# baudm/parseq

Hardware: AMD Instinct MI355X
Metric: images/sec (32x128 crops) PARSeq-S AR+refine (higher is better)
Workload: dtype bf16x3

## Files before the change

parseq_amd/csrc/decoder_attn.h:

```cpp
#pragma once
#include "common.h"

namespace pq {

constexpr int DEC_MAXL = 32;
constexpr int DEC_HD = 32;

template <typename T>
__global__ __launch_bounds__(256)
void score_table_kernel(const float* __restrict__ qself, const T* __restrict__ kvtab, float* __restrict__ stab,
                        int npos, int ntok, int E) {
    const int H = E / DEC_HD;
    const size_t total = (size_t)npos * npos * ntok * H;
    const size_t idx = (size_t)blockIdx.x * blockDim.x + threadIdx.x;
    if (idx >= total) return;
    const int h = (int)(idx % H);
    size_t r = idx / H;
    const int tok = (int)(r % ntok); r /= ntok;
    const int j = (int)(r % npos);
    const int i = (int)(r / npos);
    const float* q = qself + (size_t)i * E + h * DEC_HD;
    const T* k = kvtab + ((size_t)j * ntok + tok) * (2 * E) + h * DEC_HD;
    float s = 0.f;
#pragma unroll
// ... 246 lines not shown
__device__ __forceinline__ float f24_even(unsigned hw, unsigned lw, int i) {
    return __uint_as_float(__builtin_amdgcn_perm(hw, lw, 0x0504000cu | ((unsigned)(i & 3) << 8)));
}
__device__ __forceinline__ float f24_odd(unsigned hw, unsigned lw, int i) {
    return __uint_as_float(__builtin_amdgcn_perm(hw, lw, 0x0706000cu | ((unsigned)(i & 3) << 8)));
}
__device__ __forceinline__ void f24_unpack8(const u32x4& hi, const uint2& lo, float (&v)[8]) {
#pragma unroll
    for (int i = 0; i < 8; i += 2) {
        const unsigned lw = i < 4 ? lo.x : lo.y;
        v[i] = f24_even(hi[i >> 1], lw, i);
        v[i + 1] = f24_odd(hi[i >> 1], lw, i + 1);
    }
}

template <int E, bool QSPLIT = false>
__global__ __launch_bounds__(E)
void dec_cross_attn_ar24_kernel(const float* __restrict__ qc, const QAsm qa, const unsigned char* __restrict__ kmem, const unsigned char* __restrict__ vmem,
                                size_t plane_elems, float scale, float* __restrict__ out) {
    constexpr int H = E / DEC_HD, NK = 128, LPR = 4, KPL = 16, NL = 8;
    const int lane = threadIdx.x & 63, wid = threadIdx.x >> 6, nw = E / 64, b = blockIdx.x;
    const int kl = lane / LPR, dl = lane % LPR;
    auto over_keys_sum = [](float v) {
        v = dpp_add<0x124>(v);
        v = dpp_add<0x128>(v);
        v += __shfl_xor(v, 16, 64);
        v += __shfl_xor(v, 32, 64);
        return v;
    };
    auto over_keys_max = [](float v) {
        v = dpp_max<0x124>(v);
        v = dpp_max<0x128>(v);
        v = fmaxf(v, __shfl_xor(v, 16, 64));
        v = fmaxf(v, __shfl_xor(v, 32, 64));
        return v;
    };
    __shared__ __attribute__((aligned(16))) float qs[E];
    QOne<QSPLIT> q1;
    q_issue<QSPLIT>(qa, qc, b, E, (int)threadIdx.x, q1);
    bool first = true;
    for (int h = wid; h < H; h += nw) {
        const size_t at = (((size_t)b * H + h) * NK + kl) * DEC_HD + dl * 8;
        const unsigned char* kh = kmem + at * 2; const unsigned char* kq = kmem + plane_elems * 2 + at;
        const unsigned char* vh = vmem + at * 2; const unsigned char* vq = vmem + plane_elems * 2 + at;
        u32x4 khi[NL], vhi[NL];
        uint2 klo[NL], vlo[NL];
#pragma unroll
        for (int c = 0; c < NL; ++c) khi[c] = __builtin_nontemporal_load(reinterpret_cast<const u32x4*>(kh + (size_t)c * KPL * DEC_HD * 2));
#pragma unroll
        for (int c = 0; c < NL; ++c) { const unsigned long long t = __builtin_nontemporal_load(reinterpret_cast<const unsigned long long*>(kq + (size_t)c * KPL * DEC_HD)); klo[c] = make_uint2((unsigned)t, (unsigned)(t >> 32)); }
#pragma unroll
        for (int c = 0; c < NL; ++c) vhi[c] = __builtin_nontemporal_load(reinterpret_cast<const u32x4*>(vh + (size_t)c * KPL * DEC_HD * 2));
#pragma unroll
        for (int c = 0; c < NL; ++c) { const unsigned long long t = __builtin_nontemporal_load(reinterpret_cast<const unsigned long long*>(vq + (size_t)c * KPL * DEC_HD)); vlo[c] = make_uint2((unsigned)t, (unsigned)(t >> 32)); }
        __builtin_amdgcn_sched_barrier(0);
        if (first) {
            qs[threadIdx.x] = q_finish<QSPLIT>(qa, q1, scale);
            asm volatile("s_waitcnt lgkmcnt(0)" ::: "memory");
            __builtin_amdgcn_s_barrier();
            first = false;
        }
        float qv[8];
#pragma unroll
        for (int i = 0; i < 8; i += 4) {
            const float4 v4 = *reinterpret_cast<const float4*>(qs + h * DEC_HD + dl * 8 + i);
            qv[i] = v4.x; qv[i + 1] = v4.y; qv[i + 2] = v4.z; qv[i + 3] = v4.w;
        }
        float s[NL], mx = -INFINITY;
#pragma unroll
        for (int c = 0; c < NL; ++c) {
            float kv[8];
            f24_unpack8(khi[c], klo[c], kv);
            float d = 0.f;
#pragma unroll
            for (int i = 0; i < 8; ++i) d = fmaf(qv[i], kv[i], d);
            d = dpp_add<0xB1>(d);
            d = dpp_add<0x4E>(d);
            s[c] = d;
            mx = fmaxf(mx, d);
        }
        mx = over_keys_max(mx);
        float sum = 0.f;
#pragma unroll
        for (int c = 0; c < NL; ++c) { s[c] = expf(s[c] - mx); sum += s[c]; }
        const float inv = 1.0f / over_keys_sum(sum);
        float acc[8];
#pragma unroll
        for (int i = 0; i < 8; ++i) acc[i] = 0.f;
#pragma unroll
        for (int c = 0; c < NL; ++c) {
            const float pc = s[c] * inv;
            float vv[8];
            f24_unpack8(vhi[c], vlo[c], vv);
#pragma unroll
            for (int i = 0; i < 8; ++i) acc[i] = fmaf(pc, vv[i], acc[i]);
        }
#pragma unroll
        for (int i = 0; i < 8; ++i) acc[i] = over_keys_sum(acc[i]);
        if (kl == 0) {
            float* o = out + (size_t)b * E + h * DEC_HD + dl * 8;
            *reinterpret_cast<float4*>(o) = make_float4(acc[0], acc[1], acc[2], acc[3]);
            *reinterpret_cast<float4*>(o + 4) = make_float4(acc[4], acc[5], acc[6], acc[7]);
        }
    }
}

template <typename T>
__global__ __launch_bounds__(128)
void dec_cross_attn_multi_kernel(const float* __restrict__ qc, const T* __restrict__ kmem, const T* __restrict__ vmem,
                                 int H, int Lq, float scale, T* __restrict__ out) {
    constexpr int NK = 128, QP = DEC_MAXL;
    __shared__ float sk[NK][DEC_HD + 1];
    __shared__ float sv[DEC_HD][NK + 1];
    __shared__ float sq[QP][DEC_HD];
    __shared__ float sp[QP][NK + 1];
    const int t = threadIdx.x;
    const int bh = blockIdx.x, b = bh / H, h = bh - b * H, E = H * DEC_HD;
    const T* kg = kmem + (size_t)bh * NK * DEC_HD;
// ... 552 lines not shown
```

parseq_amd/csrc/decoder_step.h:

```cpp
#pragma once
#include "common.h"
#include "decoder_attn.h"
#include "encoder_mlp.h"

namespace pq {

constexpr int DS_ROWS = 16;
constexpr int DS_NW = 8;
#ifndef PQ_DS_RING
#define PQ_DS_RING 8
#endif
constexpr int DS_RING = PQ_DS_RING;
constexpr int DS_LA = 2;

#ifndef DS_TIMERS
#define DS_TIMERS 0
#endif
#if DS_TIMERS
#define DS_T0() const unsigned long long ds_t0 = __builtin_amdgcn_s_memtime(); unsigned ds_tk[8] = {}
#define DS_TICK(i) ds_tk[i] = (unsigned)(__builtin_amdgcn_s_memtime() - ds_t0)
#else
#define DS_T0()
#define DS_TICK(i)
#endif
// ... 445 lines not shown
    const int t = threadIdx.x;
    if (t < E) {
        float sw = 0.f, sc = 0.f, sb = 0.f;
        for (int n = 0; n < E; ++n) sw += to_f32(Wo[(size_t)n * E + t]);
        for (int k = 0; k < E; ++k) { const float w = Wq[(size_t)t * E + k]; sc = fmaf(ln_w[k], w, sc); sb = fmaf(ln_b[k], w, sb); }
        qfold[t] = sw / (float)E; qfold[E + t] = sc; qfold[2 * E + t] = sb + bq[t];
    }
    if (t < npos) {
        float s0 = 0.f;
        for (int n = 0; n < E; ++n) s0 += pos_queries[(size_t)t * E + n] + bo[n];
        qfold[3 * E + t] = s0 / (float)E;
    }
}

template <int E, bool X3 = false, int QS = 1>
__global__ __launch_bounds__(64 * DS_NW)
void dec_step_mid_kernel(int do_finish, int do_start, int pos, int M,
                         const float* __restrict__ tq, const float* __restrict__ partial, const float* __restrict__ b2,
                         const float* __restrict__ lnf_w, const float* __restrict__ lnf_b, float eps, const bf16_t* __restrict__ Wh,
                         const float* __restrict__ bh, int C, float* __restrict__ logits, int Ltot, int argmax_mode, int eos_id,
                         unsigned char* __restrict__ eos_seen, int* __restrict__ eos_rows, int* __restrict__ ar_len,
                         const float* __restrict__ stab, const typename std::conditional<X3, float, bf16_t>::type* __restrict__ kvtab, int* __restrict__ tok, int ldt, int ntok,
                         int npos, const bf16_t* __restrict__ Wo, const float* __restrict__ bo, const float* __restrict__ pos_queries,
                         const float* __restrict__ ln1_w, const float* __restrict__ ln1_b, const bf16_t* __restrict__ Wq,
                         const float* __restrict__ bq, float* __restrict__ t_out, float* __restrict__ qc_out,
                         const float* __restrict__ qfold, float* __restrict__ qstats) {
    constexpr int PA = E + 8, PT = E + 4, TILES = E / 16, TN = (TILES + DS_NW - 1) / DS_NW, PL = 128, RPW = DS_ROWS / DS_NW;
    constexpr int DS_SPLIT = ds_split<E>();
    constexpr int EN = E / QS, TS = EN / 16, TNS = (TS + DS_NW - 1) / DS_NW;
    static_assert(QS == 1 || EN % 64 == 0, "a split's columns are whole k-chunks of the fragment packs");
    constexpr int NPL = X3 ? 2 : 1, ALO = DS_ROWS * PA;
    extern __shared__ __attribute__((aligned(16))) unsigned char smem_ds[];
    bf16_t* abuf = reinterpret_cast<bf16_t*>(smem_ds);
    float* tl = reinterpret_cast<float*>(abuf + NPL * DS_ROWS * PA);
    float* lg = tl + DS_ROWS * PT;
    const int lane = threadIdx.x & 63, wave = threadIdx.x >> 6, r16 = lane & 15, g = lane >> 4;
    float* prm = lg + DS_ROWS * PL;
    float* const s_lnf_w = prm, * const s_lnf_b = prm + E, * const s_bh = prm + 2 * E, * const s_bo = prm + 2 * E + 128, * const s_posq = prm + 3 * E + 128,
         * const s_ln1_w = prm + 4 * E + 128, * const s_ln1_b = prm + 5 * E + 128, * const s_bq = prm + 6 * E + 128;
    unsigned char* wring = reinterpret_cast<unsigned char*>(prm + ds_mid_params<E>()) + wave * DS_RING * 1024;
    const int qs = QS > 1 ? (int)(blockIdx.x % QS) : 0;
    const int row0 = (int)(blockIdx.x / QS) * DS_ROWS;
    if (QS > 1 && !do_start && qs != 0) return;
    int picked[RPW], tokv[RPW];
#pragma unroll
    for (int rr = 0; rr < RPW; ++rr) {
        picked[rr] = -1;
        tokv[rr] = (do_start && lane <= pos) ? tok[(size_t)min(row0 + wave * RPW + rr, M - 1) * ldt + lane] : 0;
    }
    DS_T0();
    static_assert(E <= 64 * DS_NW, "one parameter per thread and segment");
    float* const prm_dst[8] = {s_lnf_w, s_lnf_b, s_bh, s_bo, s_posq, s_ln1_w, s_ln1_b, s_bq};
    const float* const prm_src[8] = {lnf_w, lnf_b, bh, bo, pos_queries + (size_t)min(pos, npos - 1) * E, ln1_w, QS > 1 ? qfold : ln1_b, bq};
    const float c0 = QS > 1 ? qfold[3 * E + min(pos, npos - 1)] : 0.f;
    const int prm_n[8] = {E, E, 128, E, E, E, E, E}, prm_valid[8] = {E, E, C, E, E, E, E, E};
    float prm_v[8];
    ds_params_load<8>(prm_v, prm_src, prm_valid);
// ... 169 lines not shown
        ds_wave_gemm<E, TN, true, NPL>(abuf, PA, Wq, TILES, wave, wring, acc, 0, 0, ALO);
#pragma unroll
        for (int t = 0; t < TN; ++t) {
            const int tile = wave + DS_NW * t;
            if (tile < TILES && row0 + r16 < M) {
                const int n = tile * 16 + 4 * g;
                const float4 bv = *reinterpret_cast<const float4*>(s_bq + n);
                f32x4 o = {acc[t][0] + bv.x, acc[t][1] + bv.y, acc[t][2] + bv.z, acc[t][3] + bv.w};
                *reinterpret_cast<f32x4*>(qc_out + (size_t)(row0 + r16) * E + n) = o;
            }
        }
    }
    }
#if DS_TIMERS
    DS_TICK(7);
    if (do_finish && blockIdx.x == 0 && threadIdx.x == 0) {
        float* dst = logits + (size_t)(pos - 1) * C;
        for (int i = 0; i < 8; ++i) dst[i] = (float)ds_tk[i];
        for (int i = 0; i < 5; ++i) dst[16 + i] = partial[(size_t)DS_SPLIT * M * E + i];
    }
#endif
}

template <int E, bool X3 = false>
__global__ __launch_bounds__(64 * DS_NW)
void dec_step_mlp_kernel(const typename std::conditional<X3, float, bf16_t>::type* __restrict__ ca, const float* __restrict__ t_in, const bf16_t* __restrict__ Wco,
                         const float* __restrict__ bco, const float* __restrict__ ln2_w, const float* __restrict__ ln2_b, float eps,
                         const bf16_t* __restrict__ W1, const float* __restrict__ b1, const bf16_t* __restrict__ W2,
                         float* __restrict__ tq_out, float* __restrict__ partial, int M) {
    constexpr int DS_SPLIT = ds_split<E>();
    constexpr int F = 4 * E, FS = F / DS_SPLIT, PA = E + 8, PH = FS + 8, PT = E + 4, TILES = E / 16, TN = (TILES + DS_NW - 1) / DS_NW;
    constexpr int TN1 = FS / 16 / DS_NW;
    static_assert(FS % (16 * DS_NW) == 0 && FS % 64 == 0, "hidden width must split evenly over the workgroups and waves");
    constexpr int PL = X3 ? 2 : 1, ALO = DS_ROWS * PA, HLO = DS_ROWS * PH;
    extern __shared__ __attribute__((aligned(16))) unsigned char smem_ds[];
    bf16_t* abuf = reinterpret_cast<bf16_t*>(smem_ds);
    bf16_t* hbuf = abuf + PL * DS_ROWS * PA;
    float* tl = reinterpret_cast<float*>(hbuf + PL * DS_ROWS * PH);
    const int lane = threadIdx.x & 63, wave = threadIdx.x >> 6, r16 = lane & 15, g = lane >> 4;
    float* prm = tl + DS_ROWS * PT;
    float* const s_bco = prm, * const s_ln2_w = prm + E, * const s_ln2_b = prm + 2 * E, * const s_b1 = prm + 3 * E;
    unsigned char* wring = reinterpret_cast<unsigned char*>(prm + ds_mlp_params<E>()) + wave * DS_RING * 1024;
    const int rt = blockIdx.x / DS_SPLIT, sp = blockIdx.x - rt * DS_SPLIT;
    const int row0 = rt * DS_ROWS;
    DS_T0();
    static_assert(E <= 64 * DS_NW && FS <= 64 * DS_NW, "one parameter per thread and segment");
    float* const prm_dst[4] = {s_bco, s_ln2_w, s_ln2_b, s_b1};
    const float* const prm_src[4] = {bco, ln2_w, ln2_b, b1 + sp * FS};
    const int prm_n[4] = {E, E, E, FS};
    float prm_v[4];
    ds_params_load<4>(prm_v, prm_src, prm_n);

    for (int i = threadIdx.x; i < DS_ROWS * (E / 8); i += 64 * DS_NW) {
        const int row = i / (E / 8), c = (i - row * (E / 8)) * 8;
        const int gr = min(row0 + row, M - 1);
        if constexpr (X3) {
            const f32x4* src = reinterpret_cast<const f32x4*>(ca + (size_t)gr * E + c);
            const f32x4 v0 = src[0], v1 = src[1];
            bf16x8 hi, lo;
#pragma unroll
            for (int j = 0; j < 4; ++j) {
                hi[j] = from_f32<bf16_t>(v0[j]); lo[j] = from_f32<bf16_t>(v0[j] - to_f32(hi[j]));
                hi[4 + j] = from_f32<bf16_t>(v1[j]); lo[4 + j] = from_f32<bf16_t>(v1[j] - to_f32(hi[4 + j]));
// ... 4 lines not shown
            *reinterpret_cast<bf16x8*>(abuf + row * PA + c) = *reinterpret_cast<const bf16x8*>(ca + (size_t)gr * E + c);
        }
    }
    for (int i = threadIdx.x; i < DS_ROWS * (E / 4); i += 64 * DS_NW) {
        const int row = i / (E / 4), c = (i - row * (E / 4)) * 4;
        const int gr = min(row0 + row, M - 1);
        *reinterpret_cast<f32x4*>(tl + row * PT + c) = *reinterpret_cast<const f32x4*>(t_in + (size_t)gr * E + c);
    }
    ds_params_store<4>(prm_v, prm_dst, prm_n, prm_n);
    ds_prefetch<E, TN, PL>(Wco, TILES, wave, wring);
    __syncthreads();
    DS_TICK(0);
    {
        f32x4 acc[TN] = {};
        ds_wave_gemm<E, TN, true, PL>(abuf, PA, Wco, TILES, wave, wring, acc, 0, 0, ALO);
        ds_prefetch<E, TN1, PL>(W1 + (size_t)sp * (FS / 16) * (E / 64) * (1024 * PL), FS / 16, wave, wring);
#pragma unroll
        for (int t = 0; t < TN; ++t) {
            const int tile = wave + DS_NW * t;
            if (tile < TILES) {
                const int n = tile * 16 + 4 * g;
                const float4 bv = *reinterpret_cast<const float4*>(s_bco + n);
                f32x4* p = reinterpret_cast<f32x4*>(tl + r16 * PT + n);
                f32x4 o = *p;
                o[0] += acc[t][0] + bv.x; o[1] += acc[t][1] + bv.y; o[2] += acc[t][2] + bv.z; o[3] += acc[t][3] + bv.w;
                *p = o;
                if (sp == 0 && row0 + r16 < M) *reinterpret_cast<f32x4*>(tq_out + (size_t)(row0 + r16) * E + n) = o;
            }
        }
    }
    __syncthreads();
    DS_TICK(1);
    ds_layernorm_rows<E, X3>(tl, PT, abuf, PA, s_ln2_w, s_ln2_b, eps, wave, ALO);
    __syncthreads();
    DS_TICK(2);
    {
        f32x4 acc[TN1] = {};
        ds_wave_gemm<E, TN1, true, PL>(abuf, PA, W1 + (size_t)sp * (FS / 16) * (E / 64) * (1024 * PL), FS / 16, wave, wring, acc, 0, 0, ALO);
        ds_prefetch<FS, TN, PL>(W2, TILES, wave, wring, sp * (FS / 64), F / 64);
#pragma unroll
        for (int t = 0; t < TN1; ++t) {
            const int n = (wave + DS_NW * t) * 16 + 4 * g;
            const float4 bv = *reinterpret_cast<const float4*>(s_b1 + n);
            if constexpr (X3) {
                const float o[4] = {gelu_erf(acc[t][0] + bv.x), gelu_erf(acc[t][1] + bv.y), gelu_erf(acc[t][2] + bv.z), gelu_erf(acc[t][3] + bv.w)};
                float ol[4];
#pragma unroll
                for (int j = 0; j < 4; ++j) ol[j] = o[j] - to_f32(from_f32<bf16_t>(o[j]));
                store4<bf16_t>(hbuf + r16 * PH + n, o);
                store4<bf16_t>(hbuf + HLO + r16 * PH + n, ol);
            } else {
                const float o[4] = {gelu_poly(acc[t][0] + bv.x), gelu_poly(acc[t][1] + bv.y), gelu_poly(acc[t][2] + bv.z), gelu_poly(acc[t][3] + bv.w)};
                store4<bf16_t>(hbuf + r16 * PH + n, o);
            }
        }
    }
    __syncthreads();
    DS_TICK(3);
    {
        f32x4 acc[TN] = {};
        ds_wave_gemm<FS, TN, true, PL>(hbuf, PH, W2, TILES, wave, wring, acc, sp * (FS / 64), F / 64, HLO);
        float* dst = partial + (size_t)sp * M * E;
#pragma unroll
        for (int t = 0; t < TN; ++t) {
            const int tile = wave + DS_NW * t;
            if (tile < TILES && row0 + r16 < M) {
                const int n = tile * 16 + 4 * g;
                *reinterpret_cast<f32x4*>(dst + (size_t)(row0 + r16) * E + n) = acc[t];
            }
        }
    }
#if DS_TIMERS
    DS_TICK(4);
    if (blockIdx.x == 0 && threadIdx.x == 0)
        for (int i = 0; i < 5; ++i) partial[(size_t)DS_SPLIT * M * E + i] = (float)ds_tk[i];
#endif
}

}
```

parseq_amd/csrc/lib_decode.hip:

```cpp
#include "lib_internal.h"

template <typename T_, int E_> struct TE { using T = T_; static constexpr int E = E_; };
template <typename F>
static int dispatch_t(const parseq_plan* p, F&& f) { return p->precision == PARSEQ_BF16 ? f(TE<bf16_t, 0>{}) : f(TE<float, 0>{}); }
template <typename F>
static int dispatch_te(const parseq_plan* p, F&& f) {
    return dispatch_t(p, [&](auto t) {
        using T = typename decltype(t)::T;
        switch (p->m->cfg.embed_dim) {
            case 192: return f(TE<T, 192>{});
            case 384: return f(TE<T, 384>{});
            default:  return f(TE<T, 768>{});
        }
    });
}

struct LnW { const float *g, *b; };
template <typename T> struct DecLayerW {
    LnW norm_q, norm_c, norm1, norm2;
    const T *sa_in, *sa_out, *ca_in, *ca_out, *lin1, *lin2;
    const float *sa_in_b, *sa_out_b, *ca_in_b, *ca_out_b, *lin1_b, *lin2_b;
};
template <typename T> struct DecW {
    DecLayerW<T> layer[PARSEQ_DEC_DEPTH_MAX];
// ... 29 lines not shown
}

struct DecPass {
    int B = 0, Lk = 1, i0 = 0, Lq = 1;
    int c0 = 0;
    const unsigned char* qmask = nullptr;
    const unsigned char* cmask = nullptr;
    const unsigned char* kpm = nullptr;
    float* logits = nullptr; int Ltot = 0;
    int argmax_mode = 0;
    const float* user_query = nullptr;
    bool fused_step_allowed = false;
};

enum DecStep { STEP_DEEP, STEP_FUSED, STEP_PER_OP };
struct DecRoute { DecStep step; bool qsplit; };
static DecRoute dec_route(const parseq_plan* p, bool latency) {
    const parseq_model* m = p->m;
    if (m->cfg.dec_depth > 1) return {STEP_DEEP, false};
    if (!(p->wstep[0] && p->fused_step && m->classes <= 128)) return {STEP_PER_OP, false};
    return {STEP_FUSED, latency && p->qsplit && m->tokens == 128 && m->cfg.max_label_length + 1 >= DS_QS + 2};
}

static float dec_scale() { return sqrtf(1.0f / (float)DEC_HD); }

enum CaKernel { CA_MFMA_N, CA_GENERIC, CA_AR24, CA_AR, CA_MULTI_MFMA, CA_MULTI_X3, CA_MULTI };
static int ca_route(bool half, int E, int NK, int Lq, bool kv24, int nsplit, CaKernel& kern) {
    if (nsplit && (nsplit != DS_QS || NK != 128 || Lq != 1)) return fail(PARSEQ_E_STATE, "cross-attention: split q-projection outside the AR step kernels");
    if (NK != 128) kern = half && (NK + 15) / 16 <= 16 ? CA_MFMA_N : CA_GENERIC;
    else if (Lq == 1) {
        if (kv24 && (half || E != 384)) return fail(PARSEQ_E_STATE, "cross-attention: 24-bit K / V rows but no kernel for this geometry");
        if (!kv24 && nsplit && E > 384) return fail(PARSEQ_E_STATE, "cross-attention: split q-projection at embed_dim %d", E);
        kern = kv24 ? CA_AR24 : CA_AR;
    } else if (half) kern = CA_MULTI_MFMA;
    else if (g_split) kern = CA_MULTI_X3;
    else if (kv24) return fail(PARSEQ_E_STATE, "cross-attention: 24-bit K / V rows outside the bf16x3 mode");
// ... 243 lines not shown
                               p->wstep[0], y.sa_out_b, w.pos_queries, y.norm1.g, y.norm1.b, p->wstep[1], y.ca_in_b, t, qsplit ? qp : tq, p->qfold, qstats);
            HIPCHK(hipGetLastError());
        }
        if (!do_start) break;
        CHK((run_cross_attention<TS, E>(p, s, 0, B, 1, ca, qa)));
        {
            ProfScope ps_(&p->prof, T_DEC_POST, s);
            hipLaunchKernelGGL((dec_step_mlp_kernel<E, X3>), dim3(grid.x * ds_split<E>()), block, (dec_step_mlp_lds<E, X3>()), s, ca, t, p->wstep[2],
                               y.ca_out_b, y.norm2.g, y.norm2.b, c.dec_ln_eps, p->wstep[3], y.lin1_b, p->wstep[4], tq, partial, M);
            HIPCHK(hipGetLastError());
        }
    }
    return 0;
}

template <typename T, int E>
static int forward_impl(parseq_plan* p, int B, int flags, int refine_iters, int num_steps, float* logits, int* out_len, hipStream_t s) {
    const parseq_config& c = p->m->cfg;
    const int C = p->m->classes;
    const bool ar = flags & PARSEQ_FLAG_DECODE_AR, testing = flags & PARSEQ_FLAG_TESTING;
    const DecW<T> w = dec_weights<T>(p);
    const DecRoute route = dec_route(p, flags & PARSEQ_FLAG_LATENCY);
    DecPass a; a.B = B; a.logits = logits; a.Ltot = num_steps; a.fused_step_allowed = route.step == STEP_FUSED;
    hipLaunchKernelGGL(ar_init_kernel, dim3((B * LDT + 255) / 256), dim3(256), 0, s, p->tok, LDT, B, c.bos_id, c.pad_id, p->eos_seen, p->counters, 2, num_steps);
    HIPCHK(hipGetLastError());
    bool stepwise = ar;
    if constexpr (E <= 384) {
        if (ar && route.step == STEP_FUSED) { CHK((ar_loop_fused<E, sizeof(T) == 4>(p, s, w, B, num_steps, logits, testing, route.qsplit))); stepwise = false; }
    }
    for (int i = 0; stepwise && i < num_steps; ++i) {
        a.Lk = i + 1; a.i0 = a.c0 = i; a.Lq = 1; a.argmax_mode = i + 1 < num_steps ? (testing ? 2 : 1) : 0;
        CHK((decoder_pass<T, E>(p, s, w, a)));
    }
    if (!ar) {
        a.Lk = 1; a.Lq = num_steps;
        CHK((decoder_pass<T, E>(p, s, w, a)));
    }
    for (int it = 0; it < refine_iters; ++it) {
        const int from_logits = (ar && it == 0) ? 0 : 1;
        hipLaunchKernelGGL(refine_prep_kernel, dim3((B + 3) / 4), dim3(256), 0, s, logits, num_steps, C, p->tok, LDT, p->kpm, LDT, B, c.bos_id, c.eos_id, from_logits);
        HIPCHK(hipGetLastError());
        a.Lk = a.Lq = num_steps; a.i0 = a.c0 = 0; a.qmask = a.cmask = p->cloze; a.kpm = p->kpm; a.argmax_mode = 0;
        CHK((decoder_pass<T, E>(p, s, w, a)));
// ... 159 lines not shown
```

parseq_amd/csrc/lib_internal.h:

```cpp
#pragma once
#include "../../include/parseq_hip.h"

#include <hip/hip_runtime.h>

#include <algorithm>
#include <cmath>
#include <cstdarg>
#include <cstdio>
#include <cstdlib>
#include <cstring>
#include <string>
#include <unordered_map>
#include <vector>

#include "common.h"
#include "decoder_attn.h"
#include "decoder_step.h"
#include "resize.h"
#include "encoder_attn.h"
#include "encoder_panel.h"
#include "encoder_mlp.h"
#include "encoder_attn_fused.h"
#include "encoder_blocks.h"
#include "encoder_blocks_x3.h"
#include "encoder_blocks_x3w.h"
#include "gemm.h"
#include "rowops.h"

using namespace pq;

inline thread_local char g_err[512] = "";
static int fail(int code, const char* fmt, ...) {
// ... 157 lines not shown
                                  float* __restrict__ x, int B, int Np, int E) {
    const size_t i4 = (size_t)blockIdx.x * blockDim.x + threadIdx.x;
    const size_t e4 = E / 4, per_img = (size_t)(Np + 1) * e4;
    if (i4 >= (size_t)B * per_img) return;
    const size_t b = i4 / per_img, r = i4 - b * per_img, t = r / e4, c4 = r - t * e4;
    float4 v;
    if (t == 0) {
        const float4 a = reinterpret_cast<const float4*>(cls)[c4], q = reinterpret_cast<const float4*>(pos0)[c4];
        v = make_float4(a.x + q.x, a.y + q.y, a.z + q.z, a.w + q.w);
    } else {
        v = reinterpret_cast<const float4*>(xp)[(b * Np + (t - 1)) * e4 + c4];
    }
    reinterpret_cast<float4*>(x)[i4] = v;
}

struct parseq_plan {
    parseq_model* m = nullptr;
    int max_batch = 0;
    int precision = PARSEQ_BF16;
    uint64_t packed_version = ~0ull;
    unsigned char* arena = nullptr;
    size_t arena_bytes = 0;
    parseq_release_fn arena_release = nullptr;
    void* arena_user = nullptr;
    void* wpack = nullptr;
    bf16_t* wstep[6] = {nullptr, nullptr, nullptr, nullptr, nullptr, nullptr};
    void* kvtab = nullptr;
    float* qself = nullptr;
    void* ctab_ln = nullptr;
    float* x = nullptr;
// ... 9 lines not shown
    unsigned char* qmask_user = nullptr;
    int* counters = nullptr;
    void* kmem_l[PARSEQ_DEC_DEPTH_MAX] = {};
    void* vmem_l[PARSEQ_DEC_DEPTH_MAX] = {};
    void* kvself[PARSEQ_DEC_DEPTH_MAX] = {};
    float* xc = nullptr;
    unsigned char* cmask_user = nullptr;
    int last_batch = 0;
    bool kv24 = false;
    size_t kv_plane_elems = 0;
    bool kv24_enabled = getenv("PARSEQ_NO_KV24") == nullptr;
    int num_cus = 256;
    bool fused_step = getenv("PARSEQ_NO_FUSED_STEP") == nullptr;
    float* qfold = nullptr;
    bool qsplit = getenv("PARSEQ_NO_QSPLIT") == nullptr;
    bool fused_blocks = getenv("PARSEQ_NO_FUSED_BLOCKS") == nullptr;
    bool fused_x3 = getenv("PARSEQ_NO_FUSED_X3") == nullptr;
    int small_batch_max = [] { const char* e = getenv("PARSEQ_SMALL_BATCH"); const int v = e ? atoi(e) : 64; return v < 0 ? 0 : v; }();
    bool x3_four_waves = getenv("PARSEQ_X3_FOUR_WAVES") != nullptr;
    EncBlockParams* blocks_dev = nullptr;
    std::vector<EncBlockParams> blocks_host;
    EncTailParams enc_tail{0, 0, 0, 0, nullptr, nullptr, 0};
    bool fused_tail = getenv("PARSEQ_NO_FUSED_TAIL") == nullptr;
    float* posb = nullptr;
    unsigned wpe_off = 0;
    bool fused_head = getenv("PARSEQ_NO_FUSED_HEAD") == nullptr;
    Profiler prof;
};
constexpr int LDT = 32;

// ... 157 lines not shown
```

Measured before the change: 60400.

## Fuse the AR decode loop into one kernel per row tile, stepping through all phases

Adds a kernel that runs every autoregressive step inside one launch. Each block owns 16 rows and executes the mid phase, the 24-bit cross-attention and the full MLP split (looping over FFN splits with W1 prefetch) back to back, separated by block-local barriers. The goal is to remove the per-step kernel launches and the inter-kernel dependencies for large bf16x3 batches. The cost is that the FFN splits now run serially within a block instead of across blocks, so per-step parallelism and occupancy drop. The path is gated on batch >= 512, embed_dim 384 and kv24, and the cross-attention code is factored into shared helpers.

```diff
diff --git a/parseq_amd/csrc/decoder_ar.h b/parseq_amd/csrc/decoder_ar.h
--- /dev/null
+++ b/parseq_amd/csrc/decoder_ar.h
@@ -0,0 +1,73 @@
+#pragma once
+#include "decoder_step.h"
+
+namespace pq {
+
+template <int E, bool X3> constexpr size_t dec_ar_persistent_lds() {
+    return dec_step_mid_lds<E, X3>() > dec_step_mlp_lds<E, X3>() ? dec_step_mid_lds<E, X3>() : dec_step_mlp_lds<E, X3>();
+}
+
+__device__ __forceinline__ void ds_phase_barrier() {
+    asm volatile("s_waitcnt vmcnt(0) lgkmcnt(0)" ::: "memory");
+    __syncthreads();
+}
+
+template <typename T> __device__ __forceinline__ void ds_opaque(T*& p) { asm volatile("" : "+s"(p)); }
+
+struct DecArArgs {
+    int M, num_steps, testing;
+    float* tq; float* partial; const float* b2; const float* lnf_w; const float* lnf_b; float eps; const bf16_t* Wh; const float* bh; int C;
+    float* logits; int eos_id; unsigned char* eos_seen; int* eos_rows; int* ar_len;
+    const float* stab; const float* kvtab; int* tok; int ldt, ntok, npos; const bf16_t* Wo; const float* bo; const float* pos_queries;
+    const float* ln1_w; const float* ln1_b; const bf16_t* Wq; const float* bq; float* t;
+    const unsigned char* kmem; const unsigned char* vmem; size_t plane_elems; float scale; float* ca;
+    const bf16_t* Wco; const float* bco; const float* ln2_w; const float* ln2_b; const bf16_t* W1; const float* b1; const bf16_t* W2;
+};
+
+template <int E, bool X3>
+__global__ __launch_bounds__(64 * DS_NW)
+void dec_ar_persistent_kernel(const DecArArgs a_) {
+    static_assert(X3 && E == 384, "the 24-bit cross-attention exists for the bf16x3 arithmetic at embed_dim 384");
+    static_assert(dec_ar_persistent_lds<E, X3>() <= 160 * 1024, "LDS of a compute unit");
+    static_assert((size_t)DS_ROWS * E * sizeof(float) <= dec_ar_persistent_lds<E, X3>(), "the queries of the cross-attention phase");
+    constexpr int H = E / DEC_HD, NU = DS_ROWS * H / DS_NW;
+    static_assert(DS_ROWS * H % DS_NW == 0, "every wave takes the same number of units");
+    extern __shared__ __attribute__((aligned(16))) unsigned char smem_ds[];
+    const int bid = (int)blockIdx.x, row0 = bid * DS_ROWS, M = a_.M, wave = threadIdx.x >> 6;
+    float* qs = reinterpret_cast<float*>(smem_ds);
+#pragma unroll 1
+    for (int i = 0; i <= a_.num_steps; ++i) {
+        DecArArgs a = a_;
+        ds_opaque(a.tq); ds_opaque(a.partial); ds_opaque(a.b2); ds_opaque(a.lnf_w); ds_opaque(a.lnf_b); ds_opaque(a.Wh); ds_opaque(a.bh); ds_opaque(a.logits);
+        ds_opaque(a.stab); ds_opaque(a.kvtab); ds_opaque(a.tok); ds_opaque(a.Wo); ds_opaque(a.bo); ds_opaque(a.pos_queries); ds_opaque(a.ln1_w); ds_opaque(a.ln1_b);
+        ds_opaque(a.Wq); ds_opaque(a.bq); ds_opaque(a.t); ds_opaque(a.kmem); ds_opaque(a.vmem); ds_opaque(a.ca); ds_opaque(a.Wco); ds_opaque(a.bco);
+        ds_opaque(a.ln2_w); ds_opaque(a.ln2_b); ds_opaque(a.W1); ds_opaque(a.b1); ds_opaque(a.W2);
+        const int do_finish = i > 0, do_start = i < a.num_steps;
+        ds_mid_body<E, X3, 1>(smem_ds, bid, do_finish, do_start, i, M, a.tq, a.partial, a.b2, a.lnf_w, a.lnf_b, a.eps, a.Wh, a.bh, a.C, a.logits, a.num_steps,
+                              do_start ? (a.testing ? 2 : 1) : 0, a.eos_id, a.eos_seen, a.eos_rows, a.ar_len, a.stab, a.kvtab, a.tok, a.ldt, a.ntok, a.npos,
+                              a.Wo, a.bo, a.pos_queries, a.ln1_w, a.ln1_b, a.Wq, a.bq, a.t, a.tq, nullptr, nullptr);
+        if (!do_start) break;
+        ds_phase_barrier();
+        for (int k = threadIdx.x; k < DS_ROWS * (E / 4); k += 64 * DS_NW) {
+            const int row = k / (E / 4), c = (k - row * (E / 4)) * 4;
+            const float4 v = *reinterpret_cast<const float4*>(a.tq + (size_t)min(row0 + row, M - 1) * E + c);
+            *reinterpret_cast<float4*>(qs + row * E + c) = make_float4(v.x * a.scale, v.y * a.scale, v.z * a.scale, v.w * a.scale);
+        }
+        __syncthreads();
+        {
+#pragma unroll 1
+            for (int j = 0; j < NU; ++j) {
+                const int u = wave + DS_NW * j, crop = u / H, h = u - crop * H, b = min(row0 + crop, M - 1);
+                Ca24Rows r;
+                ca24_load(r, a.kmem, a.vmem, a.plane_elems, (size_t)b * H + h);
+                __builtin_amdgcn_sched_barrier(0);
+                ca24_attend(r, qs + crop * E + h * DEC_HD, a.ca + (size_t)b * E + h * DEC_HD, row0 + crop < M);
+            }
+        }
+        ds_phase_barrier();
+        ds_mlp_body<E, X3>(smem_ds, bid, 0, ds_split<E>(), a.ca, a.t, a.Wco, a.bco, a.ln2_w, a.ln2_b, a.eps, a.W1, a.b1, a.W2, a.tq, a.partial, M);
+        ds_phase_barrier();
+    }
+}
+
+}
diff --git a/parseq_amd/csrc/decoder_attn.h b/parseq_amd/csrc/decoder_attn.h
--- a/parseq_amd/csrc/decoder_attn.h
+++ b/parseq_amd/csrc/decoder_attn.h
@@ -284,13 +284,25 @@
     }
 }
 
-template <int E, bool QSPLIT = false>
-__global__ __launch_bounds__(E)
-void dec_cross_attn_ar24_kernel(const float* __restrict__ qc, const QAsm qa, const unsigned char* __restrict__ kmem, const unsigned char* __restrict__ vmem,
-                                size_t plane_elems, float scale, float* __restrict__ out) {
-    constexpr int H = E / DEC_HD, NK = 128, LPR = 4, KPL = 16, NL = 8;
-    const int lane = threadIdx.x & 63, wid = threadIdx.x >> 6, nw = E / 64, b = blockIdx.x;
-    const int kl = lane / LPR, dl = lane % LPR;
+struct Ca24Rows { u32x4 khi[8], vhi[8]; uint2 klo[8], vlo[8]; };
+__device__ __forceinline__ void ca24_load(Ca24Rows& r, const unsigned char* __restrict__ kmem, const unsigned char* __restrict__ vmem, size_t plane_elems, size_t bh) {
+    constexpr int NK = 128, LPR = 4, KPL = 16, NL = 8;
+    const int lane = threadIdx.x & 63, kl = lane / LPR, dl = lane % LPR;
+    const size_t at = (bh * NK + kl) * DEC_HD + dl * 8;
+    const unsigned char* kh = kmem + at * 2; const unsigned char* kq = kmem + plane_elems * 2 + at;
+    const unsigned char* vh = vmem + at * 2; const unsigned char* vq = vmem + plane_elems * 2 + at;
+#pragma unroll
+    for (int c = 0; c < NL; ++c) r.khi[c] = __builtin_nontemporal_load(reinterpret_cast<const u32x4*>(kh + (size_t)c * KPL * DEC_HD * 2));
+#pragma unroll
+    for (int c = 0; c < NL; ++c) { const unsigned long long t = __builtin_nontemporal_load(reinterpret_cast<const unsigned long long*>(kq + (size_t)c * KPL * DEC_HD)); r.klo[c] = make_uint2((unsigned)t, (unsigned)(t >> 32)); }
+#pragma unroll
+    for (int c = 0; c < NL; ++c) r.vhi[c] = __builtin_nontemporal_load(reinterpret_cast<const u32x4*>(vh + (size_t)c * KPL * DEC_HD * 2));
+#pragma unroll
+    for (int c = 0; c < NL; ++c) { const unsigned long long t = __builtin_nontemporal_load(reinterpret_cast<const unsigned long long*>(vq + (size_t)c * KPL * DEC_HD)); r.vlo[c] = make_uint2((unsigned)t, (unsigned)(t >> 32)); }
+}
+__device__ __forceinline__ void ca24_attend(const Ca24Rows& r, const float* qh, float* oh, bool store) {
+    constexpr int LPR = 4, NL = 8;
+    const int lane = threadIdx.x & 63, kl = lane / LPR, dl = lane % LPR;
     auto over_keys_sum = [](float v) {
         v = dpp_add<0x124>(v);
         v = dpp_add<0x128>(v);
@@ -305,24 +317,66 @@
         v = fmaxf(v, __shfl_xor(v, 32, 64));
         return v;
     };
+    float qv[8];
+#pragma unroll
+    for (int i = 0; i < 8; i += 4) {
+        const float4 v4 = *reinterpret_cast<const float4*>(qh + dl * 8 + i);
+        qv[i] = v4.x; qv[i + 1] = v4.y; qv[i + 2] = v4.z; qv[i + 3] = v4.w;
+    }
+    float s[NL], mx = -INFINITY;
+#pragma unroll
+    for (int c = 0; c < NL; ++c) {
+        float kv[8];
+        f24_unpack8(r.khi[c], r.klo[c], kv);
+        float d = 0.f;
+#pragma unroll
+        for (int i = 0; i < 8; ++i) d = fmaf(qv[i], kv[i], d);
+        d = dpp_add<0xB1>(d);
+        d = dpp_add<0x4E>(d);
+        s[c] = d;
+        mx = fmaxf(mx, d);
+    }
+    mx = over_keys_max(mx);
+    float sum = 0.f;
+#pragma unroll
+    for (int c = 0; c < NL; ++c) { s[c] = expf(s[c] - mx); sum += s[c]; }
+    const float inv = 1.0f / over_keys_sum(sum);
+    float acc[8];
+#pragma unroll
+    for (int i = 0; i < 8; ++i) acc[i] = 0.f;
+#pragma unroll
+    for (int c = 0; c < NL; ++c) {
+        const float pc = s[c] * inv;
+        float vv[8];
+        f24_unpack8(r.vhi[c], r.vlo[c], vv);
+#pragma unroll
+        for (int i = 0; i < 8; ++i) acc[i] = fmaf(pc, vv[i], acc[i]);
+    }
+#pragma unroll
+    for (int i = 0; i < 8; ++i) acc[i] = over_keys_sum(acc[i]);
+    if (kl == 0 && store) {
+        float* o = oh + dl * 8;
+        *reinterpret_cast<float4*>(o) = make_float4(acc[0], acc[1], acc[2], acc[3]);
+        *reinterpret_cast<float4*>(o + 4) = make_float4(acc[4], acc[5], acc[6], acc[7]);
+    }
+}
+
+template <int E, bool QSPLIT = false>
+__global__ __launch_bounds__(E)
+void dec_cross_attn_ar24_kernel(const float* __restrict__ qc, const QAsm qa, const unsigned char* __restrict__ kmem, const unsigned char* __restrict__ vmem,
+                                size_t plane_elems, float scale, float* __restrict__ out) {
+    constexpr int H = E / DEC_HD;
+    const int wid = threadIdx.x >> 6, nw = E / 64, b = blockIdx.x;
     __shared__ __attribute__((aligned(16))) float qs[E];
     QOne<QSPLIT> q1;
     q_issue<QSPLIT>(qa, qc, b, E, (int)threadIdx.x, q1);
     bool first = true;
-    for (int h = wid; h < H; h += nw) {
-        const size_t at = (((size_t)b * H + h) * NK + kl) * DEC_HD + dl * 8;
-        const unsigned char* kh = kmem + at * 2; const unsigned char* kq = kmem + plane_elems * 2 + at;
-        const unsigned char* vh = vmem + at * 2; const unsigned char* vq = vmem + plane_elems * 2 + at;
-        u32x4 khi[NL], vhi[NL];
-        uint2 klo[NL], vlo[NL];
-#pragma unroll
-        for (int c = 0; c < NL; ++c) khi[c] = __builtin_nontemporal_load(reinterpret_cast<const u32x4*>(kh + (size_t)c * KPL * DEC_HD * 2));
-#pragma unroll
-        for (int c = 0; c < NL; ++c) { const unsigned long long t = __builtin_nontemporal_load(reinterpret_cast<const unsigned long long*>(kq + (size_t)c * KPL * DEC_HD)); klo[c] = make_uint2((unsigned)t, (unsigned)(t >> 32)); }
-#pragma unroll
-        for (int c = 0; c < NL; ++c) vhi[c] = __builtin_nontemporal_load(reinterpret_cast<const u32x4*>(vh + (size_t)c * KPL * DEC_HD * 2));
-#pragma unroll
-        for (int c = 0; c < NL; ++c) { const unsigned long long t = __builtin_nontemporal_load(reinterpret_cast<const unsigned long long*>(vq + (size_t)c * KPL * DEC_HD)); vlo[c] = make_uint2((unsigned)t, (unsigned)(t >> 32)); }
+    static_assert(H % nw == 0, "every wave takes the same number of heads: the barrier below is uniform");
+#pragma unroll
+    for (int j = 0; j < H / nw; ++j) {
+        const int h = wid + j * nw;
+        Ca24Rows r;
+        ca24_load(r, kmem, vmem, plane_elems, (size_t)b * H + h);
         __builtin_amdgcn_sched_barrier(0);
         if (first) {
             qs[threadIdx.x] = q_finish<QSPLIT>(qa, q1, scale);
@@ -330,48 +384,7 @@
             __builtin_amdgcn_s_barrier();
             first = false;
         }
-        float qv[8];
-#pragma unroll
-        for (int i = 0; i < 8; i += 4) {
-            const float4 v4 = *reinterpret_cast<const float4*>(qs + h * DEC_HD + dl * 8 + i);
-            qv[i] = v4.x; qv[i + 1] = v4.y; qv[i + 2] = v4.z; qv[i + 3] = v4.w;
-        }
-        float s[NL], mx = -INFINITY;
-#pragma unroll
-        for (int c = 0; c < NL; ++c) {
-            float kv[8];
-            f24_unpack8(khi[c], klo[c], kv);
-            float d = 0.f;
-#pragma unroll
-            for (int i = 0; i < 8; ++i) d = fmaf(qv[i], kv[i], d);
-            d = dpp_add<0xB1>(d);
-            d = dpp_add<0x4E>(d);
-            s[c] = d;
-            mx = fmaxf(mx, d);
-        }
-        mx = over_keys_max(mx);
-        float sum = 0.f;
-#pragma unroll
-        for (int c = 0; c < NL; ++c) { s[c] = expf(s[c] - mx); sum += s[c]; }
-        const float inv = 1.0f / over_keys_sum(sum);
-        float acc[8];
-#pragma unroll
-        for (int i = 0; i < 8; ++i) acc[i] = 0.f;
-#pragma unroll
-        for (int c = 0; c < NL; ++c) {
-            const float pc = s[c] * inv;
-            float vv[8];
-            f24_unpack8(vhi[c], vlo[c], vv);
-#pragma unroll
-            for (int i = 0; i < 8; ++i) acc[i] = fmaf(pc, vv[i], acc[i]);
-        }
-#pragma unroll
-        for (int i = 0; i < 8; ++i) acc[i] = over_keys_sum(acc[i]);
-        if (kl == 0) {
-            float* o = out + (size_t)b * E + h * DEC_HD + dl * 8;
-            *reinterpret_cast<float4*>(o) = make_float4(acc[0], acc[1], acc[2], acc[3]);
-            *reinterpret_cast<float4*>(o + 4) = make_float4(acc[4], acc[5], acc[6], acc[7]);
-        }
+        ca24_attend(r, qs + h * DEC_HD, out + (size_t)b * E + h * DEC_HD, true);
     }
 }
 
diff --git a/parseq_amd/csrc/decoder_step.h b/parseq_amd/csrc/decoder_step.h
--- a/parseq_amd/csrc/decoder_step.h
+++ b/parseq_amd/csrc/decoder_step.h
@@ -483,23 +483,22 @@
 }
 
 template <int E, bool X3 = false, int QS = 1>
-__global__ __launch_bounds__(64 * DS_NW)
-void dec_step_mid_kernel(int do_finish, int do_start, int pos, int M,
-                         const float* __restrict__ tq, const float* __restrict__ partial, const float* __restrict__ b2,
+__device__ __forceinline__
+void ds_mid_body(unsigned char* smem_ds, const int bid, int do_finish, int do_start, int pos, int M,
+                         const float* tq, const float* partial, const float* __restrict__ b2,
                          const float* __restrict__ lnf_w, const float* __restrict__ lnf_b, float eps, const bf16_t* __restrict__ Wh,
                          const float* __restrict__ bh, int C, float* __restrict__ logits, int Ltot, int argmax_mode, int eos_id,
                          unsigned char* __restrict__ eos_seen, int* __restrict__ eos_rows, int* __restrict__ ar_len,
-                         const float* __restrict__ stab, const typename std::conditional<X3, float, bf16_t>::type* __restrict__ kvtab, int* __restrict__ tok, int ldt, int ntok,
+                         const float* __restrict__ stab, const typename std::conditional<X3, float, bf16_t>::type* __restrict__ kvtab, int* tok, int ldt, int ntok,
                          int npos, const bf16_t* __restrict__ Wo, const float* __restrict__ bo, const float* __restrict__ pos_queries,
                          const float* __restrict__ ln1_w, const float* __restrict__ ln1_b, const bf16_t* __restrict__ Wq,
-                         const float* __restrict__ bq, float* __restrict__ t_out, float* __restrict__ qc_out,
-                         const float* __restrict__ qfold, float* __restrict__ qstats) {
+                         const float* __restrict__ bq, float* t_out, float* qc_out,
+                         const float* __restrict__ qfold, float* qstats) {
     constexpr int PA = E + 8, PT = E + 4, TILES = E / 16, TN = (TILES + DS_NW - 1) / DS_NW, PL = 128, RPW = DS_ROWS / DS_NW;
     constexpr int DS_SPLIT = ds_split<E>();
     constexpr int EN = E / QS, TS = EN / 16, TNS = (TS + DS_NW - 1) / DS_NW;
     static_assert(QS == 1 || EN % 64 == 0, "a split's columns are whole k-chunks of the fragment packs");
     constexpr int NPL = X3 ? 2 : 1, ALO = DS_ROWS * PA;
-    extern __shared__ __attribute__((aligned(16))) unsigned char smem_ds[];
     bf16_t* abuf = reinterpret_cast<bf16_t*>(smem_ds);
     float* tl = reinterpret_cast<float*>(abuf + NPL * DS_ROWS * PA);
     float* lg = tl + DS_ROWS * PT;
@@ -508,8 +507,8 @@
     float* const s_lnf_w = prm, * const s_lnf_b = prm + E, * const s_bh = prm + 2 * E, * const s_bo = prm + 2 * E + 128, * const s_posq = prm + 3 * E + 128,
          * const s_ln1_w = prm + 4 * E + 128, * const s_ln1_b = prm + 5 * E + 128, * const s_bq = prm + 6 * E + 128;
     unsigned char* wring = reinterpret_cast<unsigned char*>(prm + ds_mid_params<E>()) + wave * DS_RING * 1024;
-    const int qs = QS > 1 ? (int)(blockIdx.x % QS) : 0;
-    const int row0 = (int)(blockIdx.x / QS) * DS_ROWS;
+    const int qs = QS > 1 ? (int)(bid % QS) : 0;
+    const int row0 = (int)(bid / QS) * DS_ROWS;
     if (QS > 1 && !do_start && qs != 0) return;
     int picked[RPW], tokv[RPW];
 #pragma unroll
@@ -709,7 +708,7 @@
     }
 #if DS_TIMERS
     DS_TICK(7);
-    if (do_finish && blockIdx.x == 0 && threadIdx.x == 0) {
+    if (do_finish && bid == 0 && threadIdx.x == 0) {
         float* dst = logits + (size_t)(pos - 1) * C;
         for (int i = 0; i < 8; ++i) dst[i] = (float)ds_tk[i];
         for (int i = 0; i < 5; ++i) dst[16 + i] = partial[(size_t)DS_SPLIT * M * E + i];
@@ -717,18 +716,35 @@
 #endif
 }
 
+template <int E, bool X3 = false, int QS = 1>
+__global__ __launch_bounds__(64 * DS_NW)
+void dec_step_mid_kernel(int do_finish, int do_start, int pos, int M,
+                         const float* __restrict__ tq, const float* __restrict__ partial, const float* __restrict__ b2,
+                         const float* __restrict__ lnf_w, const float* __restrict__ lnf_b, float eps, const bf16_t* __restrict__ Wh,
+                         const float* __restrict__ bh, int C, float* __restrict__ logits, int Ltot, int argmax_mode, int eos_id,
+                         unsigned char* __restrict__ eos_seen, int* __restrict__ eos_rows, int* __restrict__ ar_len,
+                         const float* __restrict__ stab, const typename std::conditional<X3, float, bf16_t>::type* __restrict__ kvtab, int* __restrict__ tok, int ldt, int ntok,
+                         int npos, const bf16_t* __restrict__ Wo, const float* __restrict__ bo, const float* __restrict__ pos_queries,
+                         const float* __restrict__ ln1_w, const float* __restrict__ ln1_b, const bf16_t* __restrict__ Wq,
+                         const float* __restrict__ bq, float* __restrict__ t_out, float* __restrict__ qc_out,
+                         const float* __restrict__ qfold, float* __restrict__ qstats) {
+    extern __shared__ __attribute__((aligned(16))) unsigned char smem_ds[];
+    ds_mid_body<E, X3, QS>(smem_ds, (int)blockIdx.x, do_finish, do_start, pos, M, tq, partial, b2, lnf_w, lnf_b, eps, Wh, bh, C, logits, Ltot, argmax_mode, eos_id,
+                           eos_seen, eos_rows, ar_len, stab, kvtab, tok, ldt, ntok, npos, Wo, bo, pos_queries, ln1_w, ln1_b, Wq, bq, t_out, qc_out, qfold, qstats);
+}
+
 template <int E, bool X3 = false>
-__global__ __launch_bounds__(64 * DS_NW)
-void dec_step_mlp_kernel(const typename std::conditional<X3, float, bf16_t>::type* __restrict__ ca, const float* __restrict__ t_in, const bf16_t* __restrict__ Wco,
-                         const float* __restrict__ bco, const float* __restrict__ ln2_w, const float* __restrict__ ln2_b, float eps,
-                         const bf16_t* __restrict__ W1, const float* __restrict__ b1, const bf16_t* __restrict__ W2,
-                         float* __restrict__ tq_out, float* __restrict__ partial, int M) {
+__device__ __forceinline__
+void ds_mlp_body(unsigned char* smem_ds, const int rt, const int sp0, const int sp1,
+                 const typename std::conditional<X3, float, bf16_t>::type* ca, const float* t_in, const bf16_t* __restrict__ Wco,
+                 const float* __restrict__ bco, const float* __restrict__ ln2_w, const float* __restrict__ ln2_b, float eps,
+                 const bf16_t* __restrict__ W1, const float* __restrict__ b1, const bf16_t* __restrict__ W2,
+                 float* tq_out, float* partial, int M) {
     constexpr int DS_SPLIT = ds_split<E>();
     constexpr int F = 4 * E, FS = F / DS_SPLIT, PA = E + 8, PH = FS + 8, PT = E + 4, TILES = E / 16, TN = (TILES + DS_NW - 1) / DS_NW;
     constexpr int TN1 = FS / 16 / DS_NW;
     static_assert(FS % (16 * DS_NW) == 0 && FS % 64 == 0, "hidden width must split evenly over the workgroups and waves");
     constexpr int PL = X3 ? 2 : 1, ALO = DS_ROWS * PA, HLO = DS_ROWS * PH;
-    extern __shared__ __attribute__((aligned(16))) unsigned char smem_ds[];
     bf16_t* abuf = reinterpret_cast<bf16_t*>(smem_ds);
     bf16_t* hbuf = abuf + PL * DS_ROWS * PA;
     float* tl = reinterpret_cast<float*>(hbuf + PL * DS_ROWS * PH);
@@ -736,12 +752,11 @@
     float* prm = tl + DS_ROWS * PT;
     float* const s_bco = prm, * const s_ln2_w = prm + E, * const s_ln2_b = prm + 2 * E, * const s_b1 = prm + 3 * E;
     unsigned char* wring = reinterpret_cast<unsigned char*>(prm + ds_mlp_params<E>()) + wave * DS_RING * 1024;
-    const int rt = blockIdx.x / DS_SPLIT, sp = blockIdx.x - rt * DS_SPLIT;
     const int row0 = rt * DS_ROWS;
     DS_T0();
     static_assert(E <= 64 * DS_NW && FS <= 64 * DS_NW, "one parameter per thread and segment");
     float* const prm_dst[4] = {s_bco, s_ln2_w, s_ln2_b, s_b1};
-    const float* const prm_src[4] = {bco, ln2_w, ln2_b, b1 + sp * FS};
+    const float* const prm_src[4] = {bco, ln2_w, ln2_b, b1 + sp0 * FS};
     const int prm_n[4] = {E, E, E, FS};
     float prm_v[4];
     ds_params_load<4>(prm_v, prm_src, prm_n);
@@ -776,7 +791,7 @@
     {
         f32x4 acc[TN] = {};
         ds_wave_gemm<E, TN, true, PL>(abuf, PA, Wco, TILES, wave, wring, acc, 0, 0, ALO);
-        ds_prefetch<E, TN1, PL>(W1 + (size_t)sp * (FS / 16) * (E / 64) * (1024 * PL), FS / 16, wave, wring);
+        ds_prefetch<E, TN1, PL>(W1 + (size_t)sp0 * (FS / 16) * (E / 64) * (1024 * PL), FS / 16, wave, wring);
 #pragma unroll
         for (int t = 0; t < TN; ++t) {
             const int tile = wave + DS_NW * t;
@@ -787,7 +802,7 @@
                 f32x4 o = *p;
                 o[0] += acc[t][0] + bv.x; o[1] += acc[t][1] + bv.y; o[2] += acc[t][2] + bv.z; o[3] += acc[t][3] + bv.w;
                 *p = o;
-                if (sp == 0 && row0 + r16 < M) *reinterpret_cast<f32x4*>(tq_out + (size_t)(row0 + r16) * E + n) = o;
+                if (sp0 == 0 && row0 + r16 < M) *reinterpret_cast<f32x4*>(tq_out + (size_t)(row0 + r16) * E + n) = o;
             }
         }
     }
@@ -796,6 +811,12 @@
     ds_layernorm_rows<E, X3>(tl, PT, abuf, PA, s_ln2_w, s_ln2_b, eps, wave, ALO);
     __syncthreads();
     DS_TICK(2);
+#pragma unroll 1
+    for (int sp = sp0; sp < sp1; ++sp) {
+    if (sp != sp0) {
+        if ((int)threadIdx.x < FS) s_b1[threadIdx.x] = b1[sp * FS + threadIdx.x];
+        __syncthreads();
+    }
     {
         f32x4 acc[TN1] = {};
         ds_wave_gemm<E, TN1, true, PL>(abuf, PA, W1 + (size_t)sp * (FS / 16) * (E / 64) * (1024 * PL), FS / 16, wave, wring, acc, 0, 0, ALO);
@@ -822,6 +843,7 @@
     {
         f32x4 acc[TN] = {};
         ds_wave_gemm<FS, TN, true, PL>(hbuf, PH, W2, TILES, wave, wring, acc, sp * (FS / 64), F / 64, HLO);
+        if (sp + 1 < sp1) ds_prefetch<E, TN1, PL>(W1 + (size_t)(sp + 1) * (FS / 16) * (E / 64) * (1024 * PL), FS / 16, wave, wring);
         float* dst = partial + (size_t)sp * M * E;
 #pragma unroll
         for (int t = 0; t < TN; ++t) {
@@ -832,11 +854,23 @@
             }
         }
     }
+    }
 #if DS_TIMERS
     DS_TICK(4);
-    if (blockIdx.x == 0 && threadIdx.x == 0)
+    if (rt == 0 && sp0 == 0 && threadIdx.x == 0)
         for (int i = 0; i < 5; ++i) partial[(size_t)DS_SPLIT * M * E + i] = (float)ds_tk[i];
 #endif
 }
 
-}
+template <int E, bool X3 = false>
+__global__ __launch_bounds__(64 * DS_NW)
+void dec_step_mlp_kernel(const typename std::conditional<X3, float, bf16_t>::type* __restrict__ ca, const float* __restrict__ t_in, const bf16_t* __restrict__ Wco,
+                         const float* __restrict__ bco, const float* __restrict__ ln2_w, const float* __restrict__ ln2_b, float eps,
+                         const bf16_t* __restrict__ W1, const float* __restrict__ b1, const bf16_t* __restrict__ W2,
+                         float* __restrict__ tq_out, float* __restrict__ partial, int M) {
+    extern __shared__ __attribute__((aligned(16))) unsigned char smem_ds[];
+    const int rt = blockIdx.x / ds_split<E>(), sp = blockIdx.x - rt * ds_split<E>();
+    ds_mlp_body<E, X3>(smem_ds, rt, sp, sp + 1, ca, t_in, Wco, bco, ln2_w, ln2_b, eps, W1, b1, W2, tq_out, partial, M);
+}
+
+}
diff --git a/parseq_amd/csrc/lib_decode.hip b/parseq_amd/csrc/lib_decode.hip
--- a/parseq_amd/csrc/lib_decode.hip
+++ b/parseq_amd/csrc/lib_decode.hip
@@ -67,12 +67,14 @@
 };
 
 enum DecStep { STEP_DEEP, STEP_FUSED, STEP_PER_OP };
-struct DecRoute { DecStep step; bool qsplit; };
-static DecRoute dec_route(const parseq_plan* p, bool latency) {
+struct DecRoute { DecStep step; bool qsplit; bool persistent; };
+static DecRoute dec_route(const parseq_plan* p, bool latency, int batch = 0) {
     const parseq_model* m = p->m;
-    if (m->cfg.dec_depth > 1) return {STEP_DEEP, false};
-    if (!(p->wstep[0] && p->fused_step && m->classes <= 128)) return {STEP_PER_OP, false};
-    return {STEP_FUSED, latency && p->qsplit && m->tokens == 128 && m->cfg.max_label_length + 1 >= DS_QS + 2};
+    if (m->cfg.dec_depth > 1) return {STEP_DEEP, false, false};
+    if (!(p->wstep[0] && p->fused_step && m->classes <= 128)) return {STEP_PER_OP, false, false};
+    const bool persistent = !latency && p->ar_persistent && p->precision == PARSEQ_BF16X3 && m->cfg.embed_dim == 384 && m->tokens == 128 && p->kv24 &&
+                            batch >= p->ar_persistent_min;
+    return {STEP_FUSED, latency && p->qsplit && m->tokens == 128 && m->cfg.max_label_length + 1 >= DS_QS + 2, persistent};
 }
 
 static float dec_scale() { return sqrtf(1.0f / (float)DEC_HD); }
@@ -346,19 +348,48 @@
     return 0;
 }
 
+template <int E>
+static int ar_loop_persistent(parseq_plan* p, hipStream_t s, const DecW<float>& w, int B, int num_steps, float* logits, bool testing) {
+    const parseq_config& c = p->m->cfg;
+    const DecLayerW<float>& y = w.layer[0];
+    DecArArgs a{};
+    a.M = B; a.num_steps = num_steps; a.testing = testing ? 1 : 0;
+    a.tq = p->qc; a.partial = reinterpret_cast<float*>(p->hdn); a.b2 = y.lin2_b; a.lnf_w = w.norm.g; a.lnf_b = w.norm.b; a.eps = c.dec_ln_eps;
+    a.Wh = p->wstep[5]; a.bh = w.head_b; a.C = p->m->classes; a.logits = logits; a.eos_id = c.eos_id; a.eos_seen = p->eos_seen;
+    a.eos_rows = p->counters; a.ar_len = p->counters + 1;
+    a.stab = p->stab; a.kvtab = reinterpret_cast<const float*>(p->kvtab); a.tok = p->tok; a.ldt = LDT; a.ntok = c.num_tokens; a.npos = c.max_label_length + 1;
+    a.Wo = p->wstep[0]; a.bo = y.sa_out_b; a.pos_queries = w.pos_queries; a.ln1_w = y.norm1.g; a.ln1_b = y.norm1.b; a.Wq = p->wstep[1]; a.bq = y.ca_in_b; a.t = p->t;
+    a.kmem = reinterpret_cast<const unsigned char*>(p->kmem); a.vmem = reinterpret_cast<const unsigned char*>(p->vmem); a.plane_elems = p->kv_plane_elems;
+    a.scale = dec_scale(); a.ca = reinterpret_cast<float*>(p->ca);
+    a.Wco = p->wstep[2]; a.bco = y.ca_out_b; a.ln2_w = y.norm2.g; a.ln2_b = y.norm2.b; a.W1 = p->wstep[3]; a.b1 = y.lin1_b; a.W2 = p->wstep[4];
+    static LdsAttr attr_;
+    HIPCHK(attr_.ensure(reinterpret_cast<const void*>(dec_ar_persistent_kernel<E, true>), dec_ar_persistent_lds<E, true>()));
+    ProfScope ps_(&p->prof, T_DEC_POST, s);
+    hipLaunchKernelGGL((dec_ar_persistent_kernel<E, true>), dim3((B + DS_ROWS - 1) / DS_ROWS), dim3(64 * DS_NW), (dec_ar_persistent_lds<E, true>()), s, a);
+    HIPCHK(hipGetLastError());
+    return 0;
+}
+
 template <typename T, int E>
 static int forward_impl(parseq_plan* p, int B, int flags, int refine_iters, int num_steps, float* logits, int* out_len, hipStream_t s) {
     const parseq_config& c = p->m->cfg;
     const int C = p->m->classes;
     const bool ar = flags & PARSEQ_FLAG_DECODE_AR, testing = flags & PARSEQ_FLAG_TESTING;
     const DecW<T> w = dec_weights<T>(p);
-    const DecRoute route = dec_route(p, flags & PARSEQ_FLAG_LATENCY);
+    const DecRoute route = dec_route(p, flags & PARSEQ_FLAG_LATENCY, B);
     DecPass a; a.B = B; a.logits = logits; a.Ltot = num_steps; a.fused_step_allowed = route.step == STEP_FUSED;
     hipLaunchKernelGGL(ar_init_kernel, dim3((B * LDT + 255) / 256), dim3(256), 0, s, p->tok, LDT, B, c.bos_id, c.pad_id, p->eos_seen, p->counters, 2, num_steps);
     HIPCHK(hipGetLastError());
     bool stepwise = ar;
     if constexpr (E <= 384) {
-        if (ar && route.step == STEP_FUSED) { CHK((ar_loop_fused<E, sizeof(T) == 4>(p, s, w, B, num_steps, logits, testing, route.qsplit))); stepwise = false; }
+        if (ar && route.step == STEP_FUSED) {
+            bool done = false;
+            if constexpr (E == 384 && sizeof(T) == 4) {
+                if (route.persistent) { CHK((ar_loop_persistent<E>(p, s, w, B, num_steps, logits, testing))); done = true; }
+            }
+            if (!done) CHK((ar_loop_fused<E, sizeof(T) == 4>(p, s, w, B, num_steps, logits, testing, route.qsplit)));
+            stepwise = false;
+        }
     }
     for (int i = 0; stepwise && i < num_steps; ++i) {
         a.Lk = i + 1; a.i0 = a.c0 = i; a.Lq = 1; a.argmax_mode = i + 1 < num_steps ? (testing ? 2 : 1) : 0;
diff --git a/parseq_amd/csrc/lib_internal.h b/parseq_amd/csrc/lib_internal.h
--- a/parseq_amd/csrc/lib_internal.h
+++ b/parseq_amd/csrc/lib_internal.h
@@ -16,6 +16,7 @@
 #include "common.h"
 #include "decoder_attn.h"
 #include "decoder_step.h"
+#include "decoder_ar.h"
 #include "resize.h"
 #include "encoder_attn.h"
 #include "encoder_panel.h"
@@ -203,6 +204,7 @@
     reinterpret_cast<float4*>(x)[i4] = v;
 }
 
+constexpr int AR_PERSISTENT_MIN_BATCH = 512;
 struct parseq_plan {
     parseq_model* m = nullptr;
     int max_batch = 0;
@@ -242,6 +244,8 @@
     bool fused_step = getenv("PARSEQ_NO_FUSED_STEP") == nullptr;
     float* qfold = nullptr;
     bool qsplit = getenv("PARSEQ_NO_QSPLIT") == nullptr;
+    bool ar_persistent = getenv("PARSEQ_NO_AR_PERSISTENT") == nullptr;
+    int ar_persistent_min = [] { const char* e = getenv("PARSEQ_AR_PERSISTENT_MIN"); return e ? atoi(e) : AR_PERSISTENT_MIN_BATCH; }();
     bool fused_blocks = getenv("PARSEQ_NO_FUSED_BLOCKS") == nullptr;
     bool fused_x3 = getenv("PARSEQ_NO_FUSED_X3") == nullptr;
     int small_batch_max = [] { const char* e = getenv("PARSEQ_SMALL_BATCH"); const int v = e ? atoi(e) : 64; return v < 0 ? 0 : v; }();
```

New measurement: 61950, median of 6. +2.6%, better.
